# yunfanye/Bittorrent-with-Congestion-Control

Measured on AMD Instinct MI355X. Metric: GiB/s SHA-1 hashed (device-resident 512KiB chunks) at 1/2/4/8 MI355X, higher is better.
Workload: dtype u32

## Files before the change

bittorrent-with-congestion-control_amd/csrc/sha1_gather_walk.h:

```cpp
#pragma once
#include <stdint.h>

#if defined(__HIPCC__) || defined(__CUDACC__)
#define BT_GATHER_HD __host__ __device__ __forceinline__
#else
#define BT_GATHER_HD inline
#endif

namespace btsha1 {

struct GatherSeg {
  uint64_t off;
  uint32_t len;
  uint32_t reserved;
};
static_assert(sizeof(GatherSeg) == 16, "segment layout");

struct GatherQuad {
  uint32_t v[4];
};

struct GatherCursor {
  const uint8_t *base;
  const GatherSeg *segs;
  uint32_t nseg, ja;
  const uint8_t *pa;
  uint32_t ra, la;
  uint64_t boff;
  uint32_t lb;
  uint64_t total;
};

struct GatherPlan {
  const uint8_t *q[4];
  const uint8_t *wb;
  uint32_t sq, c;
};

struct GatherSlot {
  GatherQuad q[4], wb;
  uint32_t sq, c;
};

BT_GATHER_HD GatherSeg gather_seg(const GatherSeg *p) {
  GatherSeg s;
  __builtin_memcpy(&s, p, sizeof s);
  return s;
}

BT_GATHER_HD void gather_load_b(GatherCursor &c) {
  c.boff = 0;
  c.lb = 0;
  if (c.ja + 1 < c.nseg) {
    const GatherSeg s = gather_seg(c.segs + c.ja + 1);
    c.boff = s.off;
    c.lb = s.len;
  }
}

BT_GATHER_HD void gather_begin(GatherCursor &c, const uint8_t *base, const GatherSeg *segs, uint32_t nseg) {
  c.base = base;
  c.segs = segs;
  c.nseg = nseg;
  c.ja = 0;
  c.pa = base;
  c.ra = c.la = 0;
  c.total = 0;
  if (nseg) {
    const GatherSeg s = gather_seg(segs);
    c.pa = base + s.off;
    c.ra = c.la = s.len;
  }
  gather_load_b(c);
}

BT_GATHER_HD bool gather_regular(const GatherCursor &c) {
  return c.ra >= 64u || (c.ra >= 1u && c.la >= 16u && c.lb >= 16u && c.lb >= 64u - c.ra);
}

BT_GATHER_HD void gather_plan(GatherCursor &c, GatherPlan &p) {
  const uint32_t a = c.ra < 64u ? c.ra : 64u;
  const bool cut = a < 64u;
  const uint8_t *pb = cut ? c.base + c.boff : c.pa;
#pragma unroll
  for (uint32_t i = 0; i < 4; ++i) {
    const uint32_t lo = 16u * i;
    const uint8_t *in_a = c.pa + lo, *in_b = pb + lo - a, *win_a = c.pa + a - 16u;
    p.q[i] = lo + 16u <= a ? in_a : (lo >= a ? in_b : win_a);
  }
  p.wb = pb;
  p.c = a & 15u;
  p.sq = cut && p.c ? a >> 4 : 4u;
  const uint32_t into_b = cut ? 64u - a : 0u;
  const bool step = cut || c.ra == 64u;
  c.total += 64u;
  c.pa = step ? c.base + c.boff + into_b : c.pa + 64u;
  c.ra = step ? c.lb - into_b : c.ra - 64u;
  c.la = step ? c.lb : c.la;
  c.ja += step ? 1u : 0u;
  uint32_t jb = c.ja + 1u;
  const bool has_b = jb < c.nseg;
  jb = has_b ? jb : c.nseg - 1u;
  const GatherSeg s = gather_seg(c.segs + jb);
  c.boff = s.off;
  c.lb = has_b ? s.len : 0u;
}

BT_GATHER_HD void gather_fetch(GatherSlot &s, const GatherPlan &p) {
#pragma unroll
  for (int i = 0; i < 4; ++i) __builtin_memcpy(&s.q[i], p.q[i], 16);
  __builtin_memcpy(&s.wb, p.wb, 16);
  s.sq = p.sq;
  s.c = p.c;
}

BT_GATHER_HD uint32_t gather_sel(bool c, uint32_t a, uint32_t b) { return c ? a : b; }

BT_GATHER_HD void gather_words(uint32_t (&w)[16], const GatherSlot &s) {
  uint32_t x[8];
#pragma unroll
  for (int k = 0; k < 4; ++k) {
    uint32_t v = s.q[0].v[k];
    v = gather_sel(s.sq == 1u, s.q[1].v[k], v);
    v = gather_sel(s.sq == 2u, s.q[2].v[k], v);
    v = gather_sel(s.sq == 3u, s.q[3].v[k], v);
    x[k] = v;
    x[4 + k] = s.wb.v[k];
  }
  const uint32_t sh = 16u - s.c, bits = (sh & 3u) * 8u;
  uint32_t y[6], z[5], m[4];
#pragma unroll
  for (int k = 0; k < 6; ++k) y[k] = gather_sel(sh & 8u, x[k + 2], x[k]);
#pragma unroll
  for (int k = 0; k < 5; ++k) z[k] = gather_sel(sh & 4u, y[k + 1], y[k]);
#pragma unroll
  for (int k = 0; k < 4; ++k) m[k] = (z[k] >> bits) | ((z[k + 1] << 1) << (31u - bits));
#pragma unroll
  for (int i = 0; i < 4; ++i)
#pragma unroll
    for (int k = 0; k < 4; ++k) w[4 * i + k] = __builtin_bswap32(gather_sel(s.sq == (uint32_t)i, m[k], s.q[i].v[k]));
}

BT_GATHER_HD uint32_t gather_bytes(GatherCursor &c, uint32_t (&w)[16]) {
  uint32_t got = 0;
#pragma unroll
  for (int k = 0; k < 16; ++k) {
    uint32_t v = 0;
#pragma nounroll
    for (uint32_t b = 0; b < 4; ++b) {
      while (c.ra == 0 && c.ja + 1 < c.nseg) {
        const GatherSeg s = gather_seg(c.segs + ++c.ja);
        c.pa = c.base + s.off;
        c.ra = c.la = s.len;
      }
      if (c.ra) {
        v |= (uint32_t)*c.pa++ << (24u - 8u * b);
        --c.ra;
        ++got;
      }
    }
    w[k] = v;
  }
  c.total += got;
  gather_load_b(c);
  return got;
}

template <class Sink>
BT_GATHER_HD uint32_t gather_walk(GatherCursor &c, uint32_t (&w)[16], Sink &sink) {
  for (;;) {
    if (gather_regular(c)) {
      GatherPlan p;
      GatherSlot s0, s1;
      gather_plan(c, p);
      gather_fetch(s0, p);
      while (gather_regular(c)) {
        gather_plan(c, p);
        gather_fetch(s1, p);
        sink.fence();
        gather_words(w, s0);
        sink.block(w);
        if (!gather_regular(c)) {
          s0 = s1;
          break;
        }
        gather_plan(c, p);
        gather_fetch(s0, p);
        sink.fence();
        gather_words(w, s1);
        sink.block(w);
      }
      gather_words(w, s0);
      sink.block(w);
      continue;
    }
    const uint32_t got = gather_bytes(c, w);
    if (got < 64u) return got;
    sink.block(w);
  }
}


BT_GATHER_HD uint32_t gather_seek_seg(const uint64_t *pos, uint32_t nseg, uint64_t m, uint32_t hint) {
  uint32_t lo = hint < nseg ? hint : 0u;
  lo = pos[lo] <= m ? lo : 0u;
  uint32_t step = 1u, hi = nseg;
  while (lo + step < nseg) {
    const uint32_t k = lo + step;
    if (pos[k] > m) {
      hi = k;
      break;
    }
    lo = k;
    step += step;
  }
  while (hi - lo > 1u) {
    const uint32_t mid = lo + ((hi - lo) >> 1);
    if (pos[mid] <= m) lo = mid;
    else hi = mid;
  }
  return lo;
}

BT_GATHER_HD void gather_seek(GatherCursor &c, const uint8_t *base, const GatherSeg *segs, const uint64_t *pos,
                              uint32_t nseg, uint64_t m, uint32_t hint, uint32_t *seg) {
  const uint32_t k = gather_seek_seg(pos, nseg, m, hint);
  const GatherSeg s = gather_seg(segs + k);
  const uint32_t in = (uint32_t)(m - pos[k]);
  c.base = base;
  c.segs = segs;
  c.nseg = nseg;
  c.ja = k;
  c.pa = base + s.off + in;
  c.ra = s.len - in;
  c.la = s.len;
  c.total = m;
  gather_load_b(c);
  *seg = k;
}

BT_GATHER_HD uint32_t gather_bytes_upto(GatherCursor &c, uint32_t (&w)[16], uint32_t limit) {
  uint32_t got = 0;
#pragma unroll
  for (int j = 0; j < 16; ++j) w[j] = 0u;
#pragma nounroll
  for (uint32_t k = 0; k < 16u && got < limit; ++k) {
    uint32_t v = 0;
#pragma nounroll
    for (uint32_t b = 0; b < 4; ++b) {
      while (got < limit && c.ra == 0 && c.ja + 1 < c.nseg) {
        const GatherSeg s = gather_seg(c.segs + ++c.ja);
        c.pa = c.base + s.off;
        c.ra = c.la = s.len;
      }
      if (got < limit && c.ra) {
        v |= (uint32_t)*c.pa++ << (24u - 8u * b);
        --c.ra;
        ++got;
      }
    }
#pragma unroll
    for (uint32_t j = 0; j < 16u; ++j) w[j] = gather_sel(j == k, v, w[j]);
  }
  c.total += got;
  return got;
}

BT_GATHER_HD void gather_block_at(uint32_t (&w)[16], const uint8_t *base, const GatherSeg *segs, const uint64_t *pos,
                                  uint32_t nseg, uint64_t m, uint32_t hint, uint32_t *seg) {
  GatherCursor c;
  gather_seek(c, base, segs, pos, nseg, m, hint, seg);
  if (gather_regular(c)) {
    GatherPlan p;
    GatherSlot s;
    gather_plan(c, p);
    gather_fetch(s, p);
    gather_words(w, s);
  } else {
    gather_bytes_upto(c, w, 64u);
  }
}

BT_GATHER_HD void gather_span_at(uint32_t (&w)[16], const uint8_t *base, const GatherSeg *segs, const uint64_t *pos,
                                 uint32_t nseg, uint64_t m, uint32_t want, uint32_t hint, uint32_t *seg) {
  GatherCursor c;
  gather_seek(c, base, segs, pos, nseg, m, hint, seg);
  if (want == 64u && gather_regular(c)) {
    GatherPlan p;
    GatherSlot s;
    gather_plan(c, p);
    gather_fetch(s, p);
    gather_words(w, s);
  } else {
    gather_bytes_upto(c, w, want);
  }
}

BT_GATHER_HD void gather_tail_at(uint32_t (&w)[16], const uint8_t *base, const GatherSeg *segs, const uint64_t *pos,
                                 uint32_t nseg, uint64_t m, uint32_t r, uint32_t hint) {
#pragma unroll
  for (int k = 0; k < 16; ++k) w[k] = 0u;
  if (r == 0) return;
  GatherCursor c;
  uint32_t seg;
  gather_seek(c, base, segs, pos, nseg, m, hint, &seg);
  gather_bytes_upto(c, w, r);
}


BT_GATHER_HD uint64_t gather_total(const GatherSeg *segs, uint32_t nseg) {
  uint64_t t = 0;
  for (uint32_t j = 0; j < nseg; j += 8u) {
    uint32_t l[8];
#pragma unroll
    for (uint32_t u = 0; u < 8u; ++u) l[u] = gather_seg(segs + (j + u < nseg ? j + u : nseg - 1u)).len;
#pragma unroll
    for (uint32_t u = 0; u < 8u; ++u) t += j + u < nseg ? l[u] : 0u;
  }
  return t;
}

struct GatherStepper {
  GatherCursor c;
  GatherSlot s;
  GatherSeg d;
  uint32_t dsel;
  uint32_t ahead;
  uint64_t b;
  uint64_t nfull, nb;
  uint64_t bits;
  uint32_t r;
};

BT_GATHER_HD void gather_fetch_if(GatherStepper &st, bool go, const uint8_t *idle) {
  GatherCursor &c = st.c;
  GatherSlot &s = st.s;
  const uint32_t a = c.ra < 64u ? c.ra : 64u;
  const bool cut = a < 64u;
  const uint8_t *pb = cut ? c.base + c.boff : c.pa;
  GatherPlan p;
#pragma unroll
  for (uint32_t i = 0; i < 4; ++i) {
    const uint32_t lo = 16u * i;
    const uint8_t *in_a = c.pa + lo, *in_b = pb + lo - a, *win_a = c.pa + a - 16u;
    const uint8_t *q = lo + 16u <= a ? in_a : (lo >= a ? in_b : win_a);
    p.q[i] = go ? q : idle;
  }
  p.wb = go ? pb : idle;
  p.c = a & 15u;
  p.sq = go && cut && p.c ? a >> 4 : 4u;
  const uint32_t into_b = cut ? 64u - a : 0u;
  const bool step = go && (cut || c.ra == 64u);
  const uint64_t boff = c.boff;
  const uint32_t jb = c.ja + (step ? 2u : 1u);
  const bool has_b = go && jb < c.nseg;
  const uint32_t kb = has_b ? jb : (go ? c.nseg - 1u : 0u);
  __builtin_memcpy(&st.d, go ? (const uint8_t *)(c.segs + kb) : idle, sizeof st.d);
  st.dsel = go ? (has_b ? 2u : 1u) : 0u;
  gather_fetch(s, p);
  c.total += go ? 64u : 0u;
  c.pa = step ? c.base + boff + into_b : c.pa + (go ? 64u : 0u);
  c.ra = step ? c.lb - into_b : c.ra - (go ? 64u : 0u);
  c.la = step ? c.lb : c.la;
  c.ja += step ? 1u : 0u;
}

BT_GATHER_HD void gather_step_settle(GatherStepper &st) {
  st.c.boff = st.dsel ? st.d.off : st.c.boff;
  st.c.lb = st.dsel ? (st.dsel == 2u ? st.d.len : 0u) : st.c.lb;
  st.dsel = 0u;
}

BT_GATHER_HD void gather_step_begin(GatherStepper &st, const uint8_t *base, const GatherSeg *segs, uint32_t nseg,
                                    uint64_t len, const uint8_t *idle) {
  gather_begin(st.c, base, segs, nseg);
  st.b = 0;
  st.nfull = len >> 6;
  st.r = (uint32_t)len & 63u;
  st.nb = st.nfull + (st.r >= 56u ? 2u : 1u);
  st.bits = len * 8ull;
  const bool go = st.nfull != 0 && gather_regular(st.c);
  gather_fetch_if(st, go, idle);
  st.ahead = go ? 1u : 0u;
}

BT_GATHER_HD void gather_step(GatherStepper &st, uint32_t (&w)[16], const uint8_t *idle) {
  gather_step_settle(st);
  gather_words(w, st.s);
  if (!st.ahead) {
    const uint32_t want = st.b < st.nfull ? 64u : (st.b == st.nfull ? st.r : 0u);
    gather_bytes_upto(st.c, w, want);
    if (want) gather_load_b(st.c);
    const bool tail = st.b == st.nfull, last = st.b + 1u == st.nb;
    const uint32_t wi = st.r >> 2, mark = 0x80000000u >> ((st.r & 3u) * 8u);
#pragma unroll
    for (uint32_t j = 0; j < 16u; ++j) w[j] |= tail && j == wi ? mark : 0u;
    w[14] = last ? (uint32_t)(st.bits >> 32) : w[14];
    w[15] = last ? (uint32_t)st.bits : w[15];
  }
  ++st.b;
  const bool go = st.b < st.nfull && gather_regular(st.c);
  gather_fetch_if(st, go, idle);
  st.ahead = go ? 1u : 0u;
}

}
```

Baseline: 3290.

## Predicate gather planning and prefetch next segment descriptor in SHA-1 walk loop

Replaces the branchy plan/advance step with a predicated gather_plan_if that computes fetch pointers under a go flag. It also loads the next segment descriptor one step early and commits it in a separate settle step, so descriptor loads overlap with hashing. The loop tail is restructured so the last fetched slot is not hashed separately and extra fences are added. Risks: wasted dummy fetches when go is false, extra fences, and subtle correctness changes at the loop exit.

```diff
diff --git a/bittorrent-with-congestion-control_amd/csrc/sha1_gather_walk.h b/bittorrent-with-congestion-control_amd/csrc/sha1_gather_walk.h
--- a/bittorrent-with-congestion-control_amd/csrc/sha1_gather_walk.h
+++ b/bittorrent-with-congestion-control_amd/csrc/sha1_gather_walk.h
@@ -166,32 +166,69 @@
   return got;
 }
 
+BT_GATHER_HD void gather_plan_if(GatherCursor &c, GatherPlan &p, GatherSeg &d, bool &d_has, bool go) {
+  const uint32_t a = c.ra < 64u ? c.ra : 64u;
+  const bool cut = a < 64u;
+  const uint8_t *pb = cut ? c.base + c.boff : c.pa;
+#pragma unroll
+  for (uint32_t i = 0; i < 4; ++i) {
+    const uint32_t lo = 16u * i;
+    const uint8_t *in_a = c.pa + lo, *in_b = pb + lo - a, *win_a = c.pa + a - 16u;
+    const uint8_t *q = lo + 16u <= a ? in_a : (lo >= a ? in_b : win_a);
+    p.q[i] = go ? q : p.wb;
+  }
+  p.wb = go ? pb : p.wb;
+  p.c = a & 15u;
+  p.sq = cut && p.c ? a >> 4 : 4u;
+  const uint32_t into_b = cut ? 64u - a : 0u, adv = go ? 64u : 0u;
+  const bool step = go && (cut || c.ra == 64u);
+  c.total += adv;
+  c.pa = step ? c.base + c.boff + into_b : c.pa + adv;
+  c.ra = step ? c.lb - into_b : c.ra - adv;
+  c.la = step ? c.lb : c.la;
+  c.ja += step ? 1u : 0u;
+  uint32_t jb = c.ja + 1u;
+  d_has = jb < c.nseg;
+  jb = d_has ? jb : c.nseg - 1u;
+  d = gather_seg(c.segs + jb);
+}
+
+BT_GATHER_HD void gather_settle(GatherCursor &c, const GatherSeg &d, bool d_has) {
+  c.boff = d.off;
+  c.lb = d_has ? d.len : 0u;
+}
+
 template <class Sink>
 BT_GATHER_HD uint32_t gather_walk(GatherCursor &c, uint32_t (&w)[16], Sink &sink) {
+  GatherSlot s0, s1;
   for (;;) {
     if (gather_regular(c)) {
       GatherPlan p;
-      GatherSlot s0, s1;
-      gather_plan(c, p);
+      GatherSeg d;
+      bool d_has, go;
+      gather_plan_if(c, p, d, d_has, true);
       gather_fetch(s0, p);
-      while (gather_regular(c)) {
-        gather_plan(c, p);
+      for (;;) {
+        gather_settle(c, d, d_has);
+        go = gather_regular(c);
+        gather_plan_if(c, p, d, d_has, go);
         gather_fetch(s1, p);
         sink.fence();
         gather_words(w, s0);
         sink.block(w);
-        if (!gather_regular(c)) {
-          s0 = s1;
-          break;
-        }
-        gather_plan(c, p);
+        sink.fence();
+        if (!go) break;
+        gather_settle(c, d, d_has);
+        go = gather_regular(c);
+        gather_plan_if(c, p, d, d_has, go);
         gather_fetch(s0, p);
         sink.fence();
         gather_words(w, s1);
         sink.block(w);
+        sink.fence();
+        if (!go) break;
       }
-      gather_words(w, s0);
-      sink.block(w);
+      gather_settle(c, d, d_has);
       continue;
     }
     const uint32_t got = gather_bytes(c, w);
```

Result: no change. 3285 (-0.2%).
